# fanliaoooo/xuanpolicy

Hardware: NVIDIA B200
Metric: PPO env-steps/s (higher is better)
Workload: dtype f32

## Files before the change

xuanpolicy_b200/csrc/dense_tc.cu:

```cuda
#include <stdlib.h>
#include <string.h>

#include "common.cuh"
#include "normalize.cuh"
#include "optim.cuh"
#include "sm100.cuh"

#ifdef XB_STEP_TS
extern unsigned long long* g_xb_step_ts;
#endif

namespace xb {
namespace dense {

using namespace sm100;

#ifdef XB_DENSE_TS
static long long* g_xb_ts_host = nullptr;
#define XB_TS(role, it, ev) do { if (p.ts && blockIdx.x == 0 && (it) < 64) p.ts[((role) * 64 + (it)) * 8 + (ev)] = clock64(); } while (0)
#else
#define XB_TS(role, it, ev) do { } while (0)
#endif

constexpr int BM = 128;
// ... 887 lines not shown
            sf[N + i] = e_n_head > 0 ? e_head_w[i] : 0.f;
            sf[2 * N + i] = e_n_head > 1 ? e_head_w[N + i] : 0.f;
        }
        if (p.obs) {
            const int K = KB * BK;
            for (int i = threadIdx.x; i < 5 * K; i += kThreads) {
                const int d = i / K, kk = i - d * K;
                sf[3 * N + i] = d == 4 ? p.b0[kk] : (d < p.obs_dim ? p.W0[kk * p.obs_dim + d] : 0.f);
            }
        }
    } else {
        const int K0 = p.kb_split * BK, K1 = (KB - p.kb_split) * BK;
        for (int i = threadIdx.x; i < 256; i += kThreads) {
            sf[i] = (i < K0 && p.nh0 > 0) ? p.w2_0[i] : 0.f;
            sf[256 + i] = (i < K0 && p.nh0 > 1) ? p.w2_0[K0 + i] : 0.f;
            sf[512 + i] = (i < K1 && p.nh1 > 0) ? p.w2_1[i] : 0.f;
            sf[768 + i] = (i < K1 && p.nh1 > 1) ? p.w2_1[K1 + i] : 0.f;
        }
    }
    tc_fence_before();
    __syncthreads();
    tc_fence_after();
    uint32_t tmem_base;
    asm volatile("ld.shared.u32 %0, [%1];" : "=r"(tmem_base) : "r"(tmem_slot));
    if (threadIdx.x == 0) XB_TS(0, 62, 1);
    const bool is_producer = warp == kProducerWarp;
    if (!is_producer) {
        XB_STEP_STAMP(sts, 201);
        if (pdl_early) pdl_wait();
        XB_STEP_STAMP(sts, 202);
        pdl_trigger();
    }

    if (warp == kProducerWarp) {
        {
            const uint32_t elected = elect_one_pred();
            if (lane == 0) {
                tma_prefetch_desc(map_a0);
                tma_prefetch_desc(map_bhi);
                tma_prefetch_desc(map_blo);
                if (MODE == MODE_DGRAD) tma_prefetch_desc(map_a1);
            }
            __syncwarp();
            if (B_RES) {
                mbar_arrive_expect_tx_if(elected, bar_bfull, 2u * KB * kBTile);
                for (int kb = 0; kb < KB; ++kb) {
                    tma_load_2d_if(elected, bres + kb * kBTile, map_bhi, kb * BK, n_off, bar_bfull);
                    tma_load_2d_if(elected, bres + (KB + kb) * kBTile, map_blo, kb * BK, n_off, bar_bfull);
                }
            }
            if (pdl_early) pdl_wait();
            pdl_trigger();
            uint32_t s = 0, ph = 0, sb = 0, bph = 0, it = 0;
            for (int64_t tile = tile0; tile < n_tiles; tile += tile_step) {
                for (int kb = 0; kb < KB; ++kb, ++it) {
                    if (!(MODE == MODE_FWD && p.obs) && !(MODE == MODE_DGRAD && p.signs)) {
                        mbar_wait(bar_empty + 8 * s, ph ^ 1);
                        XB_TS(0, it, 0);
                        mbar_arrive_expect_tx_if(elected, bar_full + 8 * s, kATile);
                        const bool src1 = (MODE == MODE_DGRAD) && kb >= p.kb_split;
                        const int kcol = (src1 ? kb - p.kb_split : kb) * BK;
                        tma_load_2d_if(elected, ring + s * kATile, src1 ? map_a1 : map_a0, kcol, (int)(tile * BM), bar_full + 8 * s);
                        if (++s == (uint32_t)S) { s = 0; ph ^= 1; }
                    }
                    if (!B_RES) {
                        mbar_wait(bar_bempty + 8 * sb, bph ^ 1);
                        const uint32_t bs = b_ring + sb * 2 * kBTile;
                        mbar_arrive_expect_tx_if(elected, bar_bfull_r + 8 * sb, 2 * kBTile);
                        tma_load_2d_if(elected, bs, map_bhi, kb * BK, n_off, bar_bfull_r + 8 * sb);
                        tma_load_2d_if(elected, bs + kBTile, map_blo, kb * BK, n_off, bar_bfull_r + 8 * sb);
                        if (++sb == (uint32_t)SB) { sb = 0; bph ^= 1; }
                    }
                }
            }
        }
    } else if (warp == kMmaWarp) {
        {
            const uint32_t elected = elect_one_pred();
            const uint32_t tmem_base_u = __reduce_max_sync(0xffffffffu, tmem_base);
            if (B_RES) mbar_wait(bar_bfull, 0);
            const uint32_t dummy_bar = bar_bfull, dummy_par = B_RES ? 0u : 1u;
            uint32_t ta = 0, aph = 0, sb = 0, bph = 0, lt = 0, it = 0;
            uint32_t ready = 0;
            for (int64_t tile = tile0; tile < n_tiles; tile += tile_step, ++lt) {
                const uint32_t acc = lt & 1, tph = (lt >> 1) & 1;
                mbar_wait(bar_tempty + 8 * acc, tph ^ 1);
                const uint32_t d_tmem = tmem_base_u + acc * N;
                for (int kb = 0; kb < KB; ++kb, ++it) {
                    XB_TS(1, it, 0);
                    if (!(ready & 1)) mbar_wait(bar_conv + 8 * ta, aph);
                    if (!B_RES && !(ready & 2)) mbar_wait(bar_bfull_r + 8 * sb, bph);
                    XB_TS(1, it, 1);
                    tc_fence_after();
                    const uint32_t a_hi = tmem_base_u + kACol + ta * 64, a_lo = a_hi + 32;
                    const uint32_t b_hi = B_RES ? bres + kb * kBTile : b_ring + sb * 2 * kBTile;
                    const uint32_t b_lo = B_RES ? bres + (KB + kb) * kBTile : b_hi + kBTile;
                    const uint32_t nta = ta + 1 == kTA ? 0 : ta + 1, naph = ta + 1 == kTA ? aph ^ 1 : aph;
                    const uint32_t nsb = sb + 1 == (uint32_t)SB ? 0 : sb + 1, nbph = sb + 1 == (uint32_t)SB ? bph ^ 1 : bph;
#ifdef XB_DENSE_TS
                    ready = ts_kblock_timed((p.ts && blockIdx.x == 0 && it < 64) ? p.ts + (1 * 64 + it) * 8 : nullptr,
                                      d_tmem, a_hi, a_lo, umma_desc_sw128(b_hi, 16, 1024), umma_desc_sw128(b_lo, 16, 1024),
#else
                    ready = ts_kblock(d_tmem, a_hi, a_lo, umma_desc_sw128(b_hi, 16, 1024), umma_desc_sw128(b_lo, 16, 1024),
#endif
                                      kIdesc, kb != 0, bar_conv + 8 * nta, naph, B_RES ? dummy_bar : bar_bfull_r + 8 * nsb,
                                      B_RES ? dummy_par : nbph, bar_aempty + 8 * ta, B_RES ? 0u : bar_bempty + 8 * sb,
                                      kb == KB - 1 ? bar_tfull + 8 * acc : 0u, elected);
                    XB_TS(1, it, 3);
                    ta = nta; aph = naph;
                    if (!B_RES) { sb = nsb; bph = nbph; }
                }
            }
        }
    } else if (warp >= 4) {
        const int lq = warp & 3, ch = (warp - 4) >> 2;
        const int r = 32 * lq + lane;
        const uint32_t lane_base = (uint32_t)(32 * lq) << 16;
        uint32_t s = 0, ph = 0, ta = 0, aph = 0, it = 0;
        const bool from_bits = MODE == MODE_DGRAD && p.signs != nullptr;
        const bool from_obs = (MODE == MODE_FWD && p.obs != nullptr) || from_bits;
        const bool alt = p.alt_groups != 0;
        if (!from_obs && !alt && tile0 < n_tiles) XB_TRYWAIT_ISSUE(xb_pf, bar_full + 8 * s, ph);
        for (int64_t tile = tile0; tile < n_tiles; tile += tile_step) {
            float d00 = 0.f, d01 = 0.f, d10 = 0.f, d11 = 0.f;
            if (MODE == MODE_DGRAD) {
                const int64_t row = tile * BM + r;
                if (row < p.M) {
                    d00 = p.nh0 > 0 ? __ldg(p.dout0 + row * p.nh0) : 0.f;
                    d01 = p.nh0 > 1 ? __ldg(p.dout0 + row * p.nh0 + 1) : 0.f;
                    d10 = p.nh1 > 0 ? __ldg(p.dout1 + row * p.nh1) : 0.f;
                    d11 = p.nh1 > 1 ? __ldg(p.dout1 + row * p.nh1 + 1) : 0.f;
                }
            }
            float m0ph = 0.f, m0pl = 0.f, m0qh = 0.f, m0ql = 0.f, m1ph = 0.f, m1pl = 0.f, m1qh = 0.f, m1ql = 0.f;
            if (MODE == MODE_DGRAD && p.mask_form) {
                split_tf32(d00, m0ph, m0pl);
                split_tf32(d00 * p.slope, m0qh, m0ql);
                split_tf32(d10, m1ph, m1pl);
                split_tf32(d10 * p.slope, m1qh, m1ql);
            }
            uint32_t sw[8] = {0u, 0u, 0u, 0u, 0u, 0u, 0u, 0u};
            if (from_bits) {
                const int64_t row = tile * BM + r;
                if (row < p.M) {
                    const uint32_t* sp = p.signs + row * KB;
#pragma unroll
                    for (int j = 0; j < 8; ++j) sw[j] = j < KB ? __ldg(sp + j) : 0u;
                }
            }
            float o4[4] = {0.f, 0.f, 0.f, 0.f};
            if (MODE == MODE_FWD && from_obs) {
                const int64_t row = tile * BM + r;
                if (row < p.M) {
                    for (int i = 0; i < p.obs_dim; ++i) o4[i] = __ldg(p.obs + row * p.obs_ld + i);
                    if (p.norm_new) {
                        const double* st = row < p.norm_rows ? p.norm_new : p.norm_old;
                        for (int i = 0; i < p.obs_dim; ++i) {
                            float mean, den;
                            norm_coeffs(st, 4, i, mean, den);
                            o4[i] = norm_apply(o4[i], mean, den, p.norm_clip);
                        }
                    }
                }
            }
            for (int kb = 0; kb < KB; ++kb, ++it) {
                const uint32_t ns = s + 1 == (uint32_t)S ? 0 : s + 1, nph = s + 1 == (uint32_t)S ? ph ^ 1 : ph;
                if (alt && (it & 1u) != (uint32_t)ch) {
                    if (!from_obs) { s = ns; ph = nph; }
                    if (++ta == kTA) { ta = 0; aph ^= 1; }
                    continue;
                }
                if (alt) {
                    if (!from_obs) mbar_wait(bar_full + 8 * s, ph);
                } else if (!from_obs) {
                    uint32_t ok;
                    XB_TRYWAIT_RESULT(xb_pf, ok);
                    if (!ok) mbar_wait(bar_full + 8 * s, ph);
                }
                if (threadIdx.x == 128) XB_TS(2, it, 0);
                const uint32_t a_raw = ring + s * kATile;
                const uint32_t acol0 = tmem_base + lane_base + kACol + ta * 64;
                const int n_half = alt ? 2 : 1;
                for (int hh = 0; hh < n_half; ++hh) {
                    const int chh = alt ? hh : ch;
                    float x[16];
                    uint32_t w16 = 0u;
                    if (from_bits) {
                        if (!alt) XB_TRYWAIT_ISSUE(xb_pa, bar_aempty + 8 * ta, aph ^ 1);
                        uint32_t word = sw[0];
#pragma unroll
                        for (int j = 1; j < 8; ++j) word = kb == j ? sw[j] : word;
                        w16 = word >> (16 * chh);
                    } else if (from_obs) {
                        if (!alt) XB_TRYWAIT_ISSUE(xb_pa, bar_aempty + 8 * ta, aph ^ 1);
                        const int K = KB * BK;
                        const float* w = sf + 3 * N + kb * BK + 16 * chh;
#pragma unroll
                        for (int q = 0; q < 16; ++q) {
                            float a = w[4 * K + q];
                            a += o4[0] * w[q];
                            a += o4[1] * w[K + q];
                            a += o4[2] * w[2 * K + q];
                            a += o4[3] * w[3 * K + q];
                            x[q] = a > 0.f ? a : a * p.slope;
                        }
                        if (MODE == MODE_FWD && p.h1_out && sel == 0) {
                            const int64_t row = tile * BM + r;
                            if (row < p.M) {
                                float4* dst = reinterpret_cast<float4*>(p.h1_out + row * (int64_t)K + kb * BK + 16 * chh);
#pragma unroll
                                for (int i = 0; i < 4; ++i) dst[i] = make_float4(x[4 * i], x[4 * i + 1], x[4 * i + 2], x[4 * i + 3]);
                            }
                        }
                    } else {
                        float4 xs[4];
#pragma unroll
                        for (int i = 0; i < 4; ++i) xs[i] = lds128(a_raw + sw128_off(r, 4 * chh + i));
                        if (!alt) XB_TRYWAIT_ISSUE(xb_pa, bar_aempty + 8 * ta, aph ^ 1);
                        x[0] = xs[0].x; x[1] = xs[0].y; x[2] = xs[0].z; x[3] = xs[0].w;
                        x[4] = xs[1].x; x[5] = xs[1].y; x[6] = xs[1].z; x[7] = xs[1].w;
                        x[8] = xs[2].x; x[9] = xs[2].y; x[10] = xs[2].z; x[11] = xs[2].w;
                        x[12] = xs[3].x; x[13] = xs[3].y; x[14] = xs[3].z; x[15] = xs[3].w;
                    }
                    float hi[16], lo[16];
                    if (MODE == MODE_DGRAD && p.mask_form) {
                        const int src = kb >= p.kb_split;
                        const float ph_ = src ? m1ph : m0ph, pl_ = src ? m1pl : m0pl, qh_ = src ? m1qh : m0qh, ql_ = src ? m1ql : m0ql;
                        if (from_bits) {
#pragma unroll
                            for (int q = 0; q < 16; ++q) {
                                const bool pos = (w16 >> q) & 1u;
                                hi[q] = pos ? ph_ : qh_;
                                lo[q] = pos ? pl_ : ql_;
                            }
                        } else {
#pragma unroll
                            for (int q = 0; q < 16; ++q) {
                                const bool pos = x[q] > 0.f;
                                hi[q] = pos ? ph_ : qh_;
                                lo[q] = pos ? pl_ : ql_;
                            }
                        }
                    } else {
                        if (MODE == MODE_DGRAD) {
                            const int src = kb >= p.kb_split;
                            const float* w = sf + src * 512 + (src ? kb - p.kb_split : kb) * BK + 16 * chh;
                            const float e0 = src ? d10 : d00, e1 = src ? d11 : d01;
                            if (from_bits) {
#pragma unroll
                                for (int q = 0; q < 16; ++q) x[q] = (e0 * w[q] + e1 * w[256 + q]) * (((w16 >> q) & 1u) ? 1.f : p.slope);
                            } else {
#pragma unroll
                                for (int q = 0; q < 16; ++q) x[q] = (e0 * w[q] + e1 * w[256 + q]) * (x[q] > 0.f ? 1.f : p.slope);
                            }
                        }
#pragma unroll
                        for (int q = 0; q < 16; ++q) split_tf32(x[q], hi[q], lo[q]);
                    }
                    if (threadIdx.x == 128) XB_TS(2, it, 1);
                    if (hh == 0) {
                        if (alt) {
                            mbar_wait(bar_aempty + 8 * ta, aph ^ 1);
                        } else {
                            uint32_t ok;
                            XB_TRYWAIT_RESULT(xb_pa, ok);
                            if (!ok) mbar_wait(bar_aempty + 8 * ta, aph ^ 1);
                        }
                        if (threadIdx.x == 128) XB_TS(2, it, 2);
                        if (!from_obs && !alt) XB_TRYWAIT_ISSUE(xb_pf, bar_full + 8 * ns, nph);
                        tc_fence_after();
                    }
                    tmem_st_32x16(acol0 + 16 * chh, hi);
                    tmem_st_32x16(acol0 + 16 * chh + 32, lo);
                }
                __syncwarp();
                if (lane == 0 && !from_obs) mbar_arrive(bar_empty + 8 * s);
                tmem_st_wait();
                tc_fence_before();
                __syncwarp();
                if (lane == 0) mbar_arrive(bar_conv + 8 * ta);
                if (threadIdx.x == 128) XB_TS(2, it, 3);
                if (!from_obs) { s = ns; ph = nph; }
                if (++ta == kTA) { ta = 0; aph ^= 1; }
            }
        }
    } else {
        EpiCtx c;
        c.tmem_base = tmem_base; c.bar_tfull = bar_tfull; c.bar_tempty = bar_tempty; c.bar_h1w = bar_h1w;
        c.out_ring = out_ring; c.h1_ring = h1_ring; c.O = O; c.HB = HB;
        c.tile0 = tile0; c.tile_step = tile_step; c.n_tiles = n_tiles; c.M = p.M;
        c.map_out = map_out; c.map_h1 = map_h1; c.sf = sf; c.slope = p.slope;
        c.n_head = e_n_head; c.head_b = e_head_b; c.head_out = e_head_out;
        c.store_y = MODE != MODE_FWD || p.Y != nullptr;
        c.n_off = n_off;
        c.loss = p.loss; c.sel = sel; c.red = reinterpret_cast<double*>(misc_ptr + kLossRedOff);
        c.sign_out = (MODE == MODE_FWD && p.sign_out) ? p.sign_out + sel * (N / 32) : nullptr;
        c.sign_ld = p.sign_ld;
        c.h1_signs = (MODE == MODE_DGRAD && N == 128 && p.n_split <= 1) ? p.h1_signs : nullptr;
#ifdef XB_DENSE_TS
        c.ts = p.ts;
#endif
        if (MODE == MODE_FWD) prep_dgrad_operand(p, threadIdx.x);
        epilogue_warp<N, MODE>(c, warp, lane);
    }

    if (threadIdx.x == 0) XB_TS(0, 63, 0);
    tc_fence_before();
    __syncthreads();
    XB_STEP_STAMP(sts, 203);
    if (threadIdx.x == 0) XB_TS(0, 63, 1);
    if (warp == kMmaWarp) {
        tc_fence_after();
        tmem_dealloc<kTsTmemCols>(tmem_base);
// ... 1272 lines not shown
```

xuanpolicy_b200/csrc/env_classic.cu:

```cuda
#include "common.cuh"
#include "sample.cuh"
#include "crtrig.cuh"
#include "normalize.cuh"

namespace xb {

struct Pcg64 {
    uint64_t hi, lo, inc_hi, inc_lo;
};

__device__ __forceinline__ uint64_t pcg64_next(Pcg64& g) {
    const uint64_t MH = 0x2360ED051FC65DA4ULL, ML = 0x4385DF649FCCF645ULL;
    uint64_t lo = g.lo * ML;
    uint64_t hi = __umul64hi(g.lo, ML) + g.hi * ML + g.lo * MH;
    uint64_t nlo = lo + g.inc_lo;
    uint64_t carry = nlo < lo ? 1ULL : 0ULL;
    g.hi = hi + g.inc_hi + carry;
    g.lo = nlo;
    uint64_t x = g.hi ^ g.lo;
    unsigned rot = (unsigned)(g.hi >> 58);
    return (x >> rot) | (x << ((64u - rot) & 63u));
}
__device__ __forceinline__ double pcg64_uniform(Pcg64& g, double low, double range) {
    double u = __dmul_rn((double)(pcg64_next(g) >> 11), 1.0 / 9007199254740992.0);
// ... 218 lines not shown
            y[i] = __dadd_rn(st[i], __dmul_rn(dt6, sum));
        }
        y[0] = wrap(y[0], -kPi, kPi);
        y[1] = wrap(y[1], -kPi, kPi);
        const double v1 = 4 * kPi, v2 = 9 * kPi;
        y[2] = fmin(fmax(y[2], -v1), v1);
        y[3] = fmin(fmax(y[3], -v2), v2);
#pragma unroll
        for (int i = 0; i < 4; ++i) st[i] = y[i];
        double s0, c0, s10, c10;
        sincos_cr(st[0], &s0, &c0);
        sincos_cr(__dadd_rn(st[1], st[0]), &s10, &c10);
        terminated = __dsub_rn(-c0, c10) > 1.0;
        return terminated ? 0.0 : -1.0;
    }
};

template <class Env>
__device__ __forceinline__ void observe_row(const double (&st)[Env::S], float4 (&o)[Env::kObsVec]) {
    if constexpr (Env::kObsVec == 1) o[0] = Env::observe(st);
    else Env::observe(st, o);
}
template <class Env>
__device__ __forceinline__ void put_row(float4* dst, int64_t e, const float4 (&o)[Env::kObsVec]) {
#pragma unroll
    for (int v = 0; v < Env::kObsVec; ++v) dst[e * Env::kObsVec + v] = o[v];
}

template <class Env>
__device__ __forceinline__ Pcg64 load_rng(const uint64_t* rng, int64_t N, int64_t e) {
    return Pcg64{rng[e], rng[N + e], rng[2 * N + e], rng[3 * N + e]};
}

template <class Env>
__global__ void __launch_bounds__(128) env_reset_kernel(double* __restrict__ state, uint64_t* __restrict__ rng,
                                                         int32_t* __restrict__ elapsed, double* __restrict__ ep_score,
                                                         float4* __restrict__ obs, int n_draws, int64_t N) {
    int64_t e = (int64_t)blockIdx.x * blockDim.x + threadIdx.x;
    if (e >= N) return;
    Pcg64 g = load_rng<Env>(rng, N, e);
    double st[Env::S];
#pragma unroll
    for (int k = 0; k < Env::S; ++k) st[k] = state[k * N + e];
    for (int d = 0; d < n_draws; ++d) Env::draw(st, g);
#pragma unroll
    for (int k = 0; k < Env::S; ++k) state[k * N + e] = st[k];
    rng[e] = g.hi;
    rng[N + e] = g.lo;
    elapsed[e] = 0;
    ep_score[e] = 0.0;
    float4 o[Env::kObsVec];
    observe_row<Env>(st, o);
    put_row<Env>(obs, e, o);
}

template <class Env>
__global__ void __launch_bounds__(128)
    env_step_kernel(double* __restrict__ state, uint64_t* __restrict__ rng, int32_t* __restrict__ elapsed,
                    double* __restrict__ ep_score, const typename Env::action_t* __restrict__ actions,
                    float4* __restrict__ obs, float4* __restrict__ next_obs, float* __restrict__ rew,
                    uint8_t* __restrict__ term, uint8_t* __restrict__ trunc, float4* __restrict__ reset_obs,
                    int32_t* __restrict__ ep_step_out, double* __restrict__ ep_score_out,
                    double* __restrict__ ep_stats, int max_steps, int64_t N) {
    int64_t e = (int64_t)blockIdx.x * blockDim.x + threadIdx.x;
    if (e >= N) return;
    double st[Env::S];
#pragma unroll
    for (int k = 0; k < Env::S; ++k) st[k] = state[k * N + e];
    typename Env::action_t a = actions[e];
    int32_t el = elapsed[e];
    double score = ep_score[e];

    bool terminated;
    double reward = Env::step(st, a, terminated);
    el += 1;
    bool truncated = el >= max_steps;
    score = __dadd_rn(score, reward);

    float4 o[Env::kObsVec];
    observe_row<Env>(st, o);
    put_row<Env>(obs, e, o);
    rew[e] = (float)reward;
    term[e] = terminated ? 1 : 0;
    trunc[e] = truncated ? 1 : 0;
    ep_step_out[e] = el;
    ep_score_out[e] = score;

    if (terminated || truncated) {
        if (ep_stats) {
            atomicAdd(&ep_stats[0], 1.0);
            atomicAdd(&ep_stats[1], score);
            atomicAdd(&ep_stats[2], (double)el);
        }
        Pcg64 g = load_rng<Env>(rng, N, e);
        Env::draw(st, g);
        rng[e] = g.hi;
        rng[N + e] = g.lo;
        el = 0;
        score = 0.0;
        observe_row<Env>(st, o);
        put_row<Env>(reset_obs, e, o);
    }
    if (next_obs) put_row<Env>(next_obs, e, o);
#pragma unroll
    for (int k = 0; k < Env::S; ++k) state[k * N + e] = st[k];
    elapsed[e] = el;
    ep_score[e] = score;
}

struct RolloutStepArgs {
    const float* act_param;
    const float* logstd;
    const float* val;
    uint64_t seed;
    const uint64_t* counter_dev;
    uint64_t offset;
    double* state;
    uint64_t* rng;
    int32_t* elapsed;
    double* ep_score;
    float4* obs;
    float4* next_obs;
    float* rew;
    uint8_t* term;
    uint8_t* trunc;
    float4* reset_obs;
    int32_t* ep_step_out;
    double* ep_score_out;
    double* ep_stats;
    int max_steps;
    const float4* x_in;
    void* act_out;
    float* logp_out;
    float4* obs_row;
    float* act_row;
    float* rew_row;
    float* val_row;
    float* term_row;
    uint8_t* trunc_row;
    float* logp_row;
    const float* rew_scale;
    float rew_clip;
    const float* boot_src;
    float* boot_row;
    double* trig_cache;
    int64_t N;
    StepStats stats;
#ifdef XB_STEP_TS
    unsigned long long* ts;
#endif
};

template <class Env>
__global__ void __launch_bounds__(128) rollout_step_kernel(RolloutStepArgs a) {
#ifdef XB_STEP_TS
    unsigned long long* const ts = (blockIdx.x == 0 && threadIdx.x == 0) ? a.ts : nullptr;
    a.stats.ts = threadIdx.x == 0 ? a.ts : nullptr;
#endif
    XB_STEP_STAMP(ts, 100);
    pdl_wait();
    XB_STEP_STAMP(ts, 101);
    pdl_trigger();
    constexpr int V = Env::kObsVec, D = 4 * V;
    __shared__ double stat_smem[(2 * D + 3) * 32];
    __shared__ bool stat_flag;
    const bool with_stats = a.stats.partials != nullptr;
    double acc[2 * D + 3];
#pragma unroll
    for (int k = 0; k < 2 * D + 3; ++k) acc[k] = 0.0;
    const int64_t N = a.N;
    const int64_t e = (int64_t)blockIdx.x * blockDim.x + threadIdx.x;
    if (e < N) {
    const Philox ph = philox_setup(a.seed, a.counter_dev, a.offset);
    typename Env::action_t act;
    float logp;
    if (Env::kDiscrete) {
        act = (typename Env::action_t)sample_categorical_one(a.act_param + e * Env::kActions, Env::kActions, e, ph, &logp);
        ((int64_t*)a.act_out)[e] = (int64_t)act;
        a.act_row[e] = (float)act;
    } else {
        float x;
        logp = sample_gaussian_one(a.act_param + e, a.logstd, 1, e, ph, &x);
        act = (typename Env::action_t)x;
        ((float*)a.act_out)[e] = x;
        a.act_row[e] = x;
    }
    a.logp_out[e] = logp;
    a.logp_row[e] = logp;
    if (with_stats && a.stats.obs_state_in) {
#pragma unroll
        for (int v = 0; v < V; ++v) {
            const float4 q = a.x_in[e * V + v];
            const float in[4] = {q.x, q.y, q.z, q.w};
            float o4[4];
#pragma unroll
            for (int k = 0; k < 4; ++k) {
                const int d = 4 * v + k;
                float mean, den;
                o4[k] = 0.f;
                if (d < a.stats.dim) {
                    norm_coeffs(a.stats.obs_state_in, D, d, mean, den);
                    o4[k] = norm_apply(in[k], mean, den, a.stats.obs_clip);
                }
            }
            a.obs_row[e * V + v] = make_float4(o4[0], o4[1], o4[2], o4[3]);
        }
    } else {
#pragma unroll
        for (int v = 0; v < V; ++v) a.obs_row[e * V + v] = a.x_in[e * V + v];
    }
    a.val_row[e] = a.val[e];
    if (a.boot_row) a.boot_row[e] = a.boot_src[e];
    double st[Env::S];
#pragma unroll
    for (int k = 0; k < Env::S; ++k) st[k] = a.state[k * N + e];
    int32_t el = a.elapsed[e];
    double score = a.ep_score[e];
    bool terminated;
    double reward;
    float4 o[V];
    double sc_s = 0.0, sc_c = 0.0;
    if constexpr (Env::kTrigCache) {
        bool hit = false;
        if (a.trig_cache && a.trig_cache[e] == st[0]) {
            sc_s = a.trig_cache[N + e];
            hit = true;
        }
        if (!hit) sincos_cr(st[0], &sc_s, &sc_c);
        reward = Env::step_sc(st, act, terminated, sc_s);
        sincos_cr(st[0], &sc_s, &sc_c);
        o[0] = Env::observe_sc(st, sc_s, sc_c);
    } else {
        reward = Env::step(st, act, terminated);
        observe_row<Env>(st, o);
    }
    el += 1;
    const bool truncated = el >= a.max_steps;
    score = __dadd_rn(score, reward);
    put_row<Env>(a.obs, e, o);
    const float r32 = (float)reward;
    a.rew[e] = r32;
    a.term[e] = terminated ? 1 : 0;
    a.trunc[e] = truncated ? 1 : 0;
    a.ep_step_out[e] = el;
    a.ep_score_out[e] = score;
    if (terminated || truncated) {
        if (a.ep_stats) {
            atomicAdd(&a.ep_stats[0], 1.0);
            atomicAdd(&a.ep_stats[1], score);
            atomicAdd(&a.ep_stats[2], (double)el);
        }
        Pcg64 g = load_rng<Env>(a.rng, N, e);
        Env::draw(st, g);
        a.rng[e] = g.hi;
        a.rng[N + e] = g.lo;
        el = 0;
        score = 0.0;
        if constexpr (Env::kTrigCache) {
            sincos_cr(st[0], &sc_s, &sc_c);
            o[0] = Env::observe_sc(st, sc_s, sc_c);
        } else {
            observe_row<Env>(st, o);
        }
        put_row<Env>(a.reset_obs, e, o);
    }
    if (a.next_obs) put_row<Env>(a.next_obs, e, o);
    if constexpr (Env::kTrigCache) {
        if (a.trig_cache) {
            a.trig_cache[e] = st[0];
            a.trig_cache[N + e] = sc_s;
            a.trig_cache[2 * N + e] = sc_c;
        }
    }
#pragma unroll
    for (int k = 0; k < Env::S; ++k) a.state[k * N + e] = st[k];
    a.elapsed[e] = el;
    a.ep_score[e] = score;
    float r = r32;
    if (a.rew_scale) {
        r = r / *a.rew_scale;
        r = fminf(fmaxf(r, -a.rew_clip), a.rew_clip);
    }
    a.rew_row[e] = r;
    a.term_row[e] = terminated ? 1.0f : 0.0f;
    if (a.trunc_row) a.trunc_row[e] = truncated ? 1 : 0;
    if (with_stats) {
        if (a.stats.obs_state_in) {
#pragma unroll
            for (int v = 0; v < V; ++v) {
                const float in[4] = {o[v].x, o[v].y, o[v].z, o[v].w};
#pragma unroll
                for (int k = 0; k < 4; ++k) {
                    acc[4 * v + k] = (double)in[k];
                    acc[D + 4 * v + k] = (double)in[k] * (double)in[k];
                }
            }
        }
        if (a.stats.returns) {
            double R = ((terminated && a.stats.mask_terminal) ? 0.0 : 1.0) * a.stats.gamma * a.stats.returns[e] + (double)r32;
            if (terminated || truncated) {
                acc[2 * D] = R;
                acc[2 * D + 1] = R * R;
                acc[2 * D + 2] = 1.0;
                R = 0.0;
            }
            a.stats.returns[e] = R;
        }
    }
    }
    XB_STEP_STAMP(ts, 104);
    if (with_stats) step_stats_finish<D>(a.stats, acc, N, stat_smem, &stat_flag);
}

__global__ void sincos_kernel(const double* __restrict__ x, double* __restrict__ s, double* __restrict__ c, int64_t n) {
    int64_t i = (int64_t)blockIdx.x * blockDim.x + threadIdx.x;
    if (i < n) sincos_cr(x[i], &s[i], &c[i]);
}

static inline int env_block(int64_t N) {
    if (N <= (int64_t)kNumSMs * 32 * 2) return 32;
    if (N <= (int64_t)kNumSMs * 64 * 4) return 64;
    return 128;
}

}

using namespace xb;

#ifdef XB_STEP_TS
unsigned long long* g_xb_step_ts = nullptr;
extern "C" int xb_debug_set_step_ts(void* buf) { g_xb_step_ts = (unsigned long long*)buf; return 0; }
#endif

extern "C" int xb_env_reset(int env_kind, double* state, uint64_t* rng, int32_t* elapsed, double* ep_score,
                            float* obs, int n_draws, int64_t N, xb_stream_t stream) {
    if (N <= 0 || n_draws < 0 || !state || !rng || !elapsed || !ep_score || !obs) return XB_E_BADARG;
    cudaStream_t s = (cudaStream_t)stream;
    int block = env_block(N), grid = ceil_div_i64(N, block);
    if (env_kind == XB_ENV_CARTPOLE)
        env_reset_kernel<CartPole><<<grid, block, 0, s>>>(state, rng, elapsed, ep_score, (float4*)obs, n_draws, N);
    else if (env_kind == XB_ENV_PENDULUM)
        env_reset_kernel<Pendulum><<<grid, block, 0, s>>>(state, rng, elapsed, ep_score, (float4*)obs, n_draws, N);
    else if (env_kind == XB_ENV_MOUNTAINCAR)
        env_reset_kernel<MountainCar><<<grid, block, 0, s>>>(state, rng, elapsed, ep_score, (float4*)obs, n_draws, N);
    else if (env_kind == XB_ENV_ACROBOT)
        env_reset_kernel<Acrobot><<<grid, block, 0, s>>>(state, rng, elapsed, ep_score, (float4*)obs, n_draws, N);
    else if (env_kind == XB_ENV_MOUNTAINCAR_STACK4)
        env_reset_kernel<MountainCarStack><<<grid, block, 0, s>>>(state, rng, elapsed, ep_score, (float4*)obs, n_draws, N);
    else
        return XB_E_UNSUPPORTED;
    XB_LAUNCH_CHECK();
    return 0;
}

extern "C" int xb_env_step(int env_kind, double* state, uint64_t* rng, int32_t* elapsed, double* ep_score,
                           const void* actions, float* obs, float* next_obs, float* rew, uint8_t* term,
                           uint8_t* trunc, float* reset_obs, int32_t* ep_step_out, double* ep_score_out,
                           double* ep_stats, int max_episode_steps, int64_t N, xb_stream_t stream) {
    if (N <= 0 || !state || !rng || !elapsed || !ep_score || !actions || !obs || !rew || !term || !trunc ||
        !reset_obs || !ep_step_out || !ep_score_out)
        return XB_E_BADARG;
    cudaStream_t s = (cudaStream_t)stream;
    int block = env_block(N), grid = ceil_div_i64(N, block);
    if (env_kind == XB_ENV_CARTPOLE)
        env_step_kernel<CartPole><<<grid, block, 0, s>>>(state, rng, elapsed, ep_score, (const int64_t*)actions,
                                                         (float4*)obs, (float4*)next_obs, rew, term, trunc,
                                                         (float4*)reset_obs, ep_step_out, ep_score_out, ep_stats,
                                                         max_episode_steps, N);
    else if (env_kind == XB_ENV_PENDULUM)
        env_step_kernel<Pendulum><<<grid, block, 0, s>>>(state, rng, elapsed, ep_score, (const float*)actions,
                                                         (float4*)obs, (float4*)next_obs, rew, term, trunc,
                                                         (float4*)reset_obs, ep_step_out, ep_score_out, ep_stats,
                                                         max_episode_steps, N);
    else if (env_kind == XB_ENV_MOUNTAINCAR)
        env_step_kernel<MountainCar><<<grid, block, 0, s>>>(state, rng, elapsed, ep_score, (const int64_t*)actions,
                                                            (float4*)obs, (float4*)next_obs, rew, term, trunc,
                                                            (float4*)reset_obs, ep_step_out, ep_score_out, ep_stats,
                                                            max_episode_steps, N);
    else if (env_kind == XB_ENV_ACROBOT)
        env_step_kernel<Acrobot><<<grid, block, 0, s>>>(state, rng, elapsed, ep_score, (const int64_t*)actions,
                                                        (float4*)obs, (float4*)next_obs, rew, term, trunc,
                                                        (float4*)reset_obs, ep_step_out, ep_score_out, ep_stats,
                                                        max_episode_steps, N);
    else if (env_kind == XB_ENV_MOUNTAINCAR_STACK4)
        env_step_kernel<MountainCarStack><<<grid, block, 0, s>>>(state, rng, elapsed, ep_score, (const int64_t*)actions,
                                                                 (float4*)obs, (float4*)next_obs, rew, term, trunc,
                                                                 (float4*)reset_obs, ep_step_out, ep_score_out, ep_stats,
                                                                 max_episode_steps, N);
    else
        return XB_E_UNSUPPORTED;
    XB_LAUNCH_CHECK();
    return 0;
}

extern "C" int xb_sincos_f64(const double* x, double* s, double* c, int64_t n, xb_stream_t stream) {
    if (n <= 0 || !x || !s || !c) return XB_E_BADARG;
    sincos_kernel<<<ceil_div_i64(n, 128), 128, 0, (cudaStream_t)stream>>>(x, s, c, n);
    XB_LAUNCH_CHECK();
    return 0;
}

extern "C" int xb_rollout_step(int env_kind, const float* act_param, const float* logstd, const float* val, uint64_t seed,
                               const uint64_t* counter_dev, uint64_t offset, double* state, uint64_t* rng,
                               int32_t* elapsed, double* ep_score, float* obs, float* next_obs, float* rew, uint8_t* term,
                               uint8_t* trunc, float* reset_obs, int32_t* ep_step_out, double* ep_score_out,
                               double* ep_stats, int max_episode_steps, const float* x_in, void* act_out, float* logp_out,
                               float* obs_row, float* act_row, float* rew_row, float* val_row, float* term_row,
                               uint8_t* trunc_row, float* logp_row, const float* rew_scale, float rew_clip,
                               const float* boot_src, float* boot_row, double* trig_cache, const double* obs_state_in,
                               double* obs_state_out, int obs_dim, float obs_clip, double* ret_state, float* rew_std_io,
                               double* returns, double gamma, int mask_terminal, double* stat_partials, uint32_t* stat_ticket,
                               double* stat_sums_out, int64_t N, xb_stream_t stream) {
    if (N <= 0 || !act_param || !val || !state || !rng || !elapsed || !ep_score || !obs || !rew || !term || !trunc ||
        !reset_obs || !ep_step_out || !ep_score_out || !x_in || !act_out || !logp_out || !obs_row || !act_row ||
        !rew_row || !val_row || !term_row || !logp_row)
        return XB_E_BADARG;
    if (env_kind == XB_ENV_PENDULUM && !logstd) return XB_E_BADARG;
    if ((boot_row != nullptr) != (boot_src != nullptr)) return XB_E_BADARG;
    RolloutStepArgs a{act_param, logstd, val, seed, counter_dev, offset, state, rng, elapsed, ep_score, (float4*)obs,
                      (float4*)next_obs, rew, term, trunc, (float4*)reset_obs, ep_step_out, ep_score_out, ep_stats,
                      max_episode_steps, (const float4*)x_in, act_out, logp_out, (float4*)obs_row, act_row, rew_row,
                      val_row, term_row, trunc_row, logp_row, rew_scale, rew_clip, boot_src, boot_row, trig_cache, N, StepStats{}};
    if (stat_partials) {
        if (!stat_ticket || (!obs_state_in && !returns)) return XB_E_BADARG;
        if (obs_state_in && (obs_dim < 1 || obs_dim > 8)) return XB_E_BADARG;
        if (!stat_sums_out) {
            if (obs_state_in && (!obs_state_out || obs_state_in == obs_state_out)) return XB_E_BADARG;
            if ((ret_state != nullptr) != (returns != nullptr) || (ret_state && !rew_std_io)) return XB_E_BADARG;
        }
        a.stats = StepStats{obs_state_in, obs_state_out, obs_dim, obs_clip, ret_state, rew_std_io, returns, gamma, mask_terminal,
                            stat_partials, stat_ticket, stat_sums_out};
    }
#ifdef XB_STEP_TS
    a.ts = g_xb_step_ts;
#endif
    cudaStream_t s = (cudaStream_t)stream;
    int block = env_block(N), grid = ceil_div_i64(N, block);
    if (env_kind == XB_ENV_CARTPOLE) XB_CUDA(launch_pdl(rollout_step_kernel<CartPole>, dim3(grid), dim3(block), 0, s, true, a));
    else if (env_kind == XB_ENV_PENDULUM) XB_CUDA(launch_pdl(rollout_step_kernel<Pendulum>, dim3(grid), dim3(block), 0, s, true, a));
    else if (env_kind == XB_ENV_MOUNTAINCAR) XB_CUDA(launch_pdl(rollout_step_kernel<MountainCar>, dim3(grid), dim3(block), 0, s, true, a));
    else if (env_kind == XB_ENV_ACROBOT) XB_CUDA(launch_pdl(rollout_step_kernel<Acrobot>, dim3(grid), dim3(block), 0, s, true, a));
    else if (env_kind == XB_ENV_MOUNTAINCAR_STACK4) XB_CUDA(launch_pdl(rollout_step_kernel<MountainCarStack>, dim3(grid), dim3(block), 0, s, true, a));
    else return XB_E_UNSUPPORTED;
    XB_LAUNCH_CHECK();
    return 0;
}
```

xuanpolicy_b200/csrc/normalize.cuh:

```cuda
#pragma once
#include "common.cuh"

namespace xb {

constexpr float kNormEps = 1e-8f;

__device__ __forceinline__ void chan_merge(float mean, float var, double count, float b_mean, float b_var,
                                           double b_count, float& new_mean, float& new_var, double& new_count) {
    const double tot = count + b_count;
    const float fc = (float)count, fb = (float)b_count, ft = (float)tot;
    const float delta = b_mean - mean;
    new_mean = mean + delta * fb / ft;
    const float m_a = var * fc, m_b = b_var * fb;
    const float m2 = m_a + m_b + delta * delta * fc * fb / ft;
    new_var = m2 / ft;
    new_count = tot;
}

__device__ __forceinline__ float norm_apply(float v, float mean, float den, float clip) {
    return fminf(fmaxf((v - mean) / den, -clip), clip);
}
__device__ __forceinline__ void norm_coeffs(const double* __restrict__ state, int D, int d, float& mean, float& den) {
    mean = (float)state[d];
    den = sqrtf((float)state[D + d]) + kNormEps;
}

struct StepStats {
    const double* obs_state_in;
    double* obs_state_out;
    int dim;
    float obs_clip;
    double* ret_state;
    float* rew_std;
    double* returns;
    double gamma;
    int mask_terminal;
    double* partials;
    unsigned int* ticket;
    double* sums_out;
#ifdef XB_STEP_TS
    unsigned long long* ts;
#endif
};
constexpr int kStepStatSlots = 20;

template <int D>
__device__ __forceinline__ void merge_step_stats(const double* obs_state_in, double* obs_state_out, int dim, double* ret_state,
                                                 float* rew_std, double sum_d, double sumsq_d, double n, double r_sum,
                                                 double r_sumsq, double r_n, int tid) {
    if (tid < D && obs_state_in) {
        const int d = tid;
        float nm = (float)obs_state_in[d], nv = (float)obs_state_in[D + d];
        double new_count = obs_state_in[2 * D];
        if (d < dim) {
            const double bm = sum_d / n;
            double bv = sumsq_d / n - bm * bm;
            bv = bv > 0.0 ? bv : 0.0;
            chan_merge(nm, nv, obs_state_in[2 * D], (float)bm, (float)bv, n, nm, nv, new_count);
        }
        obs_state_out[d] = (double)nm;
        obs_state_out[D + d] = (double)nv;
        if (d == 0) obs_state_out[2 * D] = obs_state_in[2 * D] + n;
    }
    if (tid == 0 && ret_state) {
        if (r_n > 0.0) {
            const double bm = r_sum / r_n;
            double bv = r_sumsq / r_n - bm * bm;
            bv = bv > 0.0 ? bv : 0.0;
            const double count = ret_state[2], tot = count + r_n, delta = bm - ret_state[0];
            const double m2 = ret_state[1] * count + bv * r_n + delta * delta * count * r_n / tot;
            ret_state[0] = ret_state[0] + delta * r_n / tot;
            ret_state[1] = m2 / tot;
            ret_state[2] = tot;
        }
        *rew_std = (float)fmin(fmax(sqrt(ret_state[1]), 0.1), 100.0);
    }
}

__device__ __forceinline__ void merge_step_sums(const double* sums, int D, const double* obs_state_in, double* obs_state_out, int dim,
                                                double* ret_state, float* rew_std, int tid) {
    const int d = tid < D ? tid : 0;
    if (D == 8)
        merge_step_stats<8>(obs_state_in, obs_state_out, dim, ret_state, rew_std, sums[d], sums[8 + d], sums[16], sums[17], sums[18],
                            sums[19], tid);
    else
        merge_step_stats<4>(obs_state_in, obs_state_out, dim, ret_state, rew_std, sums[d], sums[4 + d], sums[8], sums[9], sums[10],
                            sums[11], tid);
}

__device__ __forceinline__ double row_sum32(const double* row, int rot) {
    double a[4] = {0.0, 0.0, 0.0, 0.0};
#pragma unroll
    for (int j = 0; j < 32; j += 4) {
#pragma unroll
        for (int q = 0; q < 4; ++q) a[q] += row[(j + q + rot) & 31];
    }
    return (a[0] + a[1]) + (a[2] + a[3]);
}

__device__ __forceinline__ unsigned int ticket_take(unsigned int* ticket) {
    unsigned int old;
    asm volatile("atom.acq_rel.gpu.global.add.u32 %0, [%1], 1;" : "=r"(old) : "l"(ticket) : "memory");
    return old;
}

template <int D>
__device__ __forceinline__ void step_stats_finish(const StepStats& s, double (&acc)[2 * D + 3], int64_t N, double* smem,
                                                  bool* flag) {
    constexpr int K = 2 * D + 3;
    constexpr unsigned kFull = 0xffffffffu;
    const int lane = threadIdx.x & 31;
    double* mine = s.partials + (int64_t)blockIdx.x * kStepStatSlots;
    if (blockDim.x == 32) {
#pragma unroll
        for (int k = 0; k < K; ++k) smem[k * 32 + lane] = acc[k];
        __syncwarp();
        const double v = lane < K ? row_sum32(smem + lane * 32, lane) : 0.0;
        __syncwarp();
        if (lane < K) smem[lane] = v;
        __syncwarp();
        if (lane == 0) {
#pragma unroll
            for (int k = 0; k < K; ++k) mine[k] = smem[k];
            *flag = (ticket_take(s.ticket) == gridDim.x - 1);
        }
        __syncwarp();
    } else {
        block_sum<K>(acc, smem);
        if (threadIdx.x == 0) {
#pragma unroll
            for (int k = 0; k < K; ++k) mine[k] = acc[k];
            *flag = (ticket_take(s.ticket) == gridDim.x - 1);
        }
        __syncthreads();
    }
    if (!*flag) return;
    if (threadIdx.x >= 32) return;
    XB_STEP_STAMP(s.ts, 102);
    const int d = lane < D ? lane : 0;
    double st_mean = 0.0, st_var = 0.0, st_count = 0.0, r_mean = 0.0, r_var = 0.0, r_count = 0.0;
    if (s.obs_state_in && !s.sums_out) {
        st_mean = s.obs_state_in[d];
        st_var = s.obs_state_in[D + d];
        st_count = s.obs_state_in[2 * D];
    }
    if (s.ret_state && !s.sums_out) {
        r_mean = s.ret_state[0];
        r_var = s.ret_state[1];
        r_count = s.ret_state[2];
    }
    XB_STEP_STAMP(s.ts, 105);
    const int grid = gridDim.x;
    double t[K];
#pragma unroll
    for (int k = 0; k < K; ++k) t[k] = 0.0;
    constexpr int U = D <= 4 ? 4 : 2;
    for (int b0 = lane; b0 < grid; b0 += 32 * U) {
        double u[U][K];
#pragma unroll
        for (int j = 0; j < U; ++j) {
            const int b = b0 + 32 * j;
            const double* p = s.partials + (int64_t)(b < grid ? b : 0) * kStepStatSlots;
#pragma unroll
            for (int k = 0; k < K; ++k) u[j][k] = b < grid ? __ldcg(p + k) : 0.0;
        }
#pragma unroll
        for (int j = 0; j < U; ++j)
#pragma unroll
            for (int k = 0; k < K; ++k) t[k] += u[j][k];
    }
    __syncwarp();
#pragma unroll
    for (int k = 0; k < K; ++k) smem[k * 32 + lane] = t[k];
    __syncwarp();
    const double tot = lane < K ? row_sum32(smem + lane * 32, lane) : 0.0;
    XB_STEP_STAMP(s.ts, 106);
    if (s.sums_out) {
        if (lane < 2 * D) s.sums_out[lane] = tot;
        else if (lane < K) s.sums_out[lane + 1] = tot;
        if (lane == 0) s.sums_out[2 * D] = (double)N;
    } else {
        const double sum_d = __shfl_sync(kFull, tot, d), sumsq_d = __shfl_sync(kFull, tot, D + d);
        const double r_sum = __shfl_sync(kFull, tot, 2 * D), r_sumsq = __shfl_sync(kFull, tot, 2 * D + 1);
        const double r_n = __shfl_sync(kFull, tot, 2 * D + 2);
        if (lane < D && s.obs_state_in) {
            const double n = (double)N;
            float nm = (float)st_mean, nv = (float)st_var;
            double new_count = st_count;
            if (lane < s.dim) {
                const double bm = sum_d / n;
                double bv = sumsq_d / n - bm * bm;
                bv = bv > 0.0 ? bv : 0.0;
                chan_merge(nm, nv, st_count, (float)bm, (float)bv, n, nm, nv, new_count);
            }
            s.obs_state_out[lane] = (double)nm;
            s.obs_state_out[D + lane] = (double)nv;
            if (lane == 0) s.obs_state_out[2 * D] = st_count + n;
        }
        if (lane == 16 && s.ret_state) {
            if (r_n > 0.0) {
                const double bm = r_sum / r_n;
                double bv = r_sumsq / r_n - bm * bm;
                bv = bv > 0.0 ? bv : 0.0;
                const double tot_n = r_count + r_n, delta = bm - r_mean;
                const double m2 = r_var * r_count + bv * r_n + delta * delta * r_count * r_n / tot_n;
                r_mean = r_mean + delta * r_n / tot_n;
                r_var = m2 / tot_n;
                s.ret_state[0] = r_mean;
                s.ret_state[1] = r_var;
                s.ret_state[2] = tot_n;
            }
            *s.rew_std = (float)fmin(fmax(sqrt(r_var), 0.1), 100.0);
        }
    }
    XB_STEP_STAMP(s.ts, 107);
    if (lane == 0) *s.ticket = 0u;
    XB_STEP_STAMP(s.ts, 103);
}

}
```

Before: 50.00 million.

## Hoist env-step loads ahead of sampling and transpose stat partials layout

The rollout step kernel now issues all of its global loads up front: action params, inputs, normalization stats, state, RNG, trig cache, reward scale and previous return. This lets their latencies overlap, and launch bounds ask for 4 blocks per SM. The per-block stat partials are stored slot-major (k*grid + block) so the final reduction reads them coalesced across lanes. The dense forward loads observation normalization stats once into registers. Trade-offs: more register pressure, and the RNG state is loaded on every step even when no reset happens.

```diff
diff --git a/xuanpolicy_b200/csrc/dense_tc.cu b/xuanpolicy_b200/csrc/dense_tc.cu
--- a/xuanpolicy_b200/csrc/dense_tc.cu
+++ b/xuanpolicy_b200/csrc/dense_tc.cu
@@ -1063,13 +1063,22 @@
             if (MODE == MODE_FWD && from_obs) {
                 const int64_t row = tile * BM + r;
                 if (row < p.M) {
-                    for (int i = 0; i < p.obs_dim; ++i) o4[i] = __ldg(p.obs + row * p.obs_ld + i);
-                    if (p.norm_new) {
-                        const double* st = row < p.norm_rows ? p.norm_new : p.norm_old;
-                        for (int i = 0; i < p.obs_dim; ++i) {
-                            float mean, den;
-                            norm_coeffs(st, 4, i, mean, den);
-                            o4[i] = norm_apply(o4[i], mean, den, p.norm_clip);
+                    const double* st = p.norm_new ? (row < p.norm_rows ? p.norm_new : p.norm_old) : nullptr;
+                    double st_mean[4], st_var[4];
+#pragma unroll
+                    for (int i = 0; i < 4; ++i) {
+                        const bool on = i < p.obs_dim;
+                        o4[i] = on ? __ldg(p.obs + row * p.obs_ld + i) : 0.f;
+                        st_mean[i] = on && st ? st[i] : 0.0;
+                        st_var[i] = on && st ? st[4 + i] : 0.0;
+                    }
+                    if (st) {
+#pragma unroll
+                        for (int i = 0; i < 4; ++i) {
+                            if (i < p.obs_dim) {
+                                const float mean = (float)st_mean[i], den = sqrtf((float)st_var[i]) + kNormEps;
+                                o4[i] = norm_apply(o4[i], mean, den, p.norm_clip);
+                            }
                         }
                     }
                 }
diff --git a/xuanpolicy_b200/csrc/env_classic.cu b/xuanpolicy_b200/csrc/env_classic.cu
--- a/xuanpolicy_b200/csrc/env_classic.cu
+++ b/xuanpolicy_b200/csrc/env_classic.cu
@@ -394,7 +394,7 @@
 };
 
 template <class Env>
-__global__ void __launch_bounds__(128) rollout_step_kernel(RolloutStepArgs a) {
+__global__ void __launch_bounds__(128, 4) rollout_step_kernel(RolloutStepArgs a) {
 #ifdef XB_STEP_TS
     unsigned long long* const ts = (blockIdx.x == 0 && threadIdx.x == 0) ? a.ts : nullptr;
     a.stats.ts = threadIdx.x == 0 ? a.ts : nullptr;
@@ -414,34 +414,62 @@
     const int64_t e = (int64_t)blockIdx.x * blockDim.x + threadIdx.x;
     if (e < N) {
     const Philox ph = philox_setup(a.seed, a.counter_dev, a.offset);
+    constexpr int A = Env::kDiscrete ? Env::kActions : 1;
+    float prm[A];
+#pragma unroll
+    for (int j = 0; j < A; ++j) prm[j] = a.act_param[e * A + j];
+    const float ls = Env::kDiscrete ? 0.f : a.logstd[0];
+    float4 xin[V];
+#pragma unroll
+    for (int v = 0; v < V; ++v) xin[v] = a.x_in[e * V + v];
+    const bool norm_in = with_stats && a.stats.obs_state_in;
+    double nst[2 * D];
+#pragma unroll
+    for (int d = 0; d < 2 * D; ++d) nst[d] = norm_in ? a.stats.obs_state_in[d] : 0.0;
+    const float val = a.val[e];
+    const float boot = a.boot_row ? a.boot_src[e] : 0.f;
+    double st[Env::S];
+#pragma unroll
+    for (int k = 0; k < Env::S; ++k) st[k] = a.state[k * N + e];
+    int32_t el = a.elapsed[e];
+    double score = a.ep_score[e];
+    Pcg64 g = load_rng<Env>(a.rng, N, e);
+    double tc_key = 0.0, tc_s = 0.0;
+    if constexpr (Env::kTrigCache) {
+        if (a.trig_cache) {
+            tc_key = a.trig_cache[e];
+            tc_s = a.trig_cache[N + e];
+        }
+    }
+    const float rew_scale = a.rew_scale ? *a.rew_scale : 1.f;
+    const double ret_prev = (with_stats && a.stats.returns) ? a.stats.returns[e] : 0.0;
     typename Env::action_t act;
     float logp;
     if (Env::kDiscrete) {
-        act = (typename Env::action_t)sample_categorical_one(a.act_param + e * Env::kActions, Env::kActions, e, ph, &logp);
+        act = (typename Env::action_t)sample_categorical_one(prm, Env::kActions, e, ph, &logp);
         ((int64_t*)a.act_out)[e] = (int64_t)act;
         a.act_row[e] = (float)act;
     } else {
         float x;
-        logp = sample_gaussian_one(a.act_param + e, a.logstd, 1, e, ph, &x);
+        logp = sample_gaussian_one(prm, &ls, 1, e, ph, &x);
         act = (typename Env::action_t)x;
         ((float*)a.act_out)[e] = x;
         a.act_row[e] = x;
     }
     a.logp_out[e] = logp;
     a.logp_row[e] = logp;
-    if (with_stats && a.stats.obs_state_in) {
+    if (norm_in) {
 #pragma unroll
         for (int v = 0; v < V; ++v) {
-            const float4 q = a.x_in[e * V + v];
+            const float4 q = xin[v];
             const float in[4] = {q.x, q.y, q.z, q.w};
             float o4[4];
 #pragma unroll
             for (int k = 0; k < 4; ++k) {
                 const int d = 4 * v + k;
-                float mean, den;
                 o4[k] = 0.f;
                 if (d < a.stats.dim) {
-                    norm_coeffs(a.stats.obs_state_in, D, d, mean, den);
+                    const float mean = (float)nst[d], den = sqrtf((float)nst[D + d]) + kNormEps;
                     o4[k] = norm_apply(in[k], mean, den, a.stats.obs_clip);
                 }
             }
@@ -449,23 +477,18 @@
         }
     } else {
 #pragma unroll
-        for (int v = 0; v < V; ++v) a.obs_row[e * V + v] = a.x_in[e * V + v];
-    }
-    a.val_row[e] = a.val[e];
-    if (a.boot_row) a.boot_row[e] = a.boot_src[e];
-    double st[Env::S];
-#pragma unroll
-    for (int k = 0; k < Env::S; ++k) st[k] = a.state[k * N + e];
-    int32_t el = a.elapsed[e];
-    double score = a.ep_score[e];
+        for (int v = 0; v < V; ++v) a.obs_row[e * V + v] = xin[v];
+    }
+    a.val_row[e] = val;
+    if (a.boot_row) a.boot_row[e] = boot;
     bool terminated;
     double reward;
     float4 o[V];
     double sc_s = 0.0, sc_c = 0.0;
     if constexpr (Env::kTrigCache) {
         bool hit = false;
-        if (a.trig_cache && a.trig_cache[e] == st[0]) {
-            sc_s = a.trig_cache[N + e];
+        if (a.trig_cache && tc_key == st[0]) {
+            sc_s = tc_s;
             hit = true;
         }
         if (!hit) sincos_cr(st[0], &sc_s, &sc_c);
@@ -492,7 +515,6 @@
             atomicAdd(&a.ep_stats[1], score);
             atomicAdd(&a.ep_stats[2], (double)el);
         }
-        Pcg64 g = load_rng<Env>(a.rng, N, e);
         Env::draw(st, g);
         a.rng[e] = g.hi;
         a.rng[N + e] = g.lo;
@@ -520,7 +542,7 @@
     a.ep_score[e] = score;
     float r = r32;
     if (a.rew_scale) {
-        r = r / *a.rew_scale;
+        r = r / rew_scale;
         r = fminf(fmaxf(r, -a.rew_clip), a.rew_clip);
     }
     a.rew_row[e] = r;
@@ -539,7 +561,7 @@
             }
         }
         if (a.stats.returns) {
-            double R = ((terminated && a.stats.mask_terminal) ? 0.0 : 1.0) * a.stats.gamma * a.stats.returns[e] + (double)r32;
+            double R = ((terminated && a.stats.mask_terminal) ? 0.0 : 1.0) * a.stats.gamma * ret_prev + (double)r32;
             if (terminated || truncated) {
                 acc[2 * D] = R;
                 acc[2 * D + 1] = R * R;
diff --git a/xuanpolicy_b200/csrc/normalize.cuh b/xuanpolicy_b200/csrc/normalize.cuh
--- a/xuanpolicy_b200/csrc/normalize.cuh
+++ b/xuanpolicy_b200/csrc/normalize.cuh
@@ -110,7 +110,8 @@
     constexpr int K = 2 * D + 3;
     constexpr unsigned kFull = 0xffffffffu;
     const int lane = threadIdx.x & 31;
-    double* mine = s.partials + (int64_t)blockIdx.x * kStepStatSlots;
+    const int grid = gridDim.x;
+    double* mine = s.partials + blockIdx.x;
     if (blockDim.x == 32) {
 #pragma unroll
         for (int k = 0; k < K; ++k) smem[k * 32 + lane] = acc[k];
@@ -121,7 +122,7 @@
         __syncwarp();
         if (lane == 0) {
 #pragma unroll
-            for (int k = 0; k < K; ++k) mine[k] = smem[k];
+            for (int k = 0; k < K; ++k) mine[(int64_t)k * grid] = smem[k];
             *flag = (ticket_take(s.ticket) == gridDim.x - 1);
         }
         __syncwarp();
@@ -129,7 +130,7 @@
         block_sum<K>(acc, smem);
         if (threadIdx.x == 0) {
 #pragma unroll
-            for (int k = 0; k < K; ++k) mine[k] = acc[k];
+            for (int k = 0; k < K; ++k) mine[(int64_t)k * grid] = acc[k];
             *flag = (ticket_take(s.ticket) == gridDim.x - 1);
         }
         __syncthreads();
@@ -150,7 +151,6 @@
         r_count = s.ret_state[2];
     }
     XB_STEP_STAMP(s.ts, 105);
-    const int grid = gridDim.x;
     double t[K];
 #pragma unroll
     for (int k = 0; k < K; ++k) t[k] = 0.0;
@@ -160,9 +160,9 @@
 #pragma unroll
         for (int j = 0; j < U; ++j) {
             const int b = b0 + 32 * j;
-            const double* p = s.partials + (int64_t)(b < grid ? b : 0) * kStepStatSlots;
-#pragma unroll
-            for (int k = 0; k < K; ++k) u[j][k] = b < grid ? __ldcg(p + k) : 0.0;
+            const double* p = s.partials + (b < grid ? b : 0);
+#pragma unroll
+            for (int k = 0; k < K; ++k) u[j][k] = b < grid ? __ldcg(p + (int64_t)k * grid) : 0.0;
         }
 #pragma unroll
         for (int j = 0; j < U; ++j)
```

New measurement: 50.81 million, median of 6. +1.6%, better.
